# krlong014/PySolvers

Hardware: AMD Instinct MI355X
Metric: CG iterations/sec + SpMV GB/s vs HBM roofline, 5-pt Laplacian N=10M (higher is better)
Workload: dtype f64

## Files before the change

### include/psk_lab.h

```cpp
#ifndef PSK_LAB_H
#define PSK_LAB_H

#include "psk.h"

#ifdef __cplusplus
extern "C" {
#endif

int psk_lab_occupy_begin(int32_t wgs, int32_t lds_bytes, double seconds);
int psk_lab_occupy_end(int32_t *timed_out);
int psk_lab_dispatch_probe(int32_t nwg, int32_t lds_bytes, double usec, int64_t *rec_out);
int psk_lab_occupy_xcc(int32_t *counts);
int psk_lab_trisolve_workers(const psk_prec *M, int32_t which, int32_t *enrolled, int32_t *grid);
int psk_lab_trisolve_plan(int64_t n, const int32_t *rowptr, const int32_t *colidx, const double *vals, int32_t upper,
                          int32_t unit, const int32_t *nat, int32_t num_cus, int64_t syncfree_waves, int32_t *schedule,
                          double *est, int64_t *info);
int psk_lab_dist_plan(int64_t n_global, const int64_t *row_starts, int32_t P, int32_t rank, const int64_t *rowptr,
                      const int32_t *colidx, int32_t *lcol, int64_t *halo, int64_t *nhalo, int32_t *pack, int64_t *npack,
                      int64_t *peers, int32_t *npeers);
int psk_lab_amg_gs_pair(psk_prec *M, int32_t set, int32_t *levels_on, int32_t *levels_eligible);
int psk_lab_spmv_rotate(const psk_csr *A, const double *const *xs, double *const *ys, int32_t nbuf, int32_t reps,
                        int32_t dot, double *avg_ms);
int psk_lab_spmv_after_write(const psk_csr *A, double *x, double *y, const double *src, double *scratch,
                             int32_t target, int32_t reps, int32_t dot, double *avg_ms);
int psk_lab_cheby_ab(const psk_prec *M, const double *v, int32_t reps, double *fused_ms, double *pieces_ms);
int psk_lab_pcg_stagger(int32_t *blocks, int32_t *ring);
int psk_lab_pcg_staggers(const psk_csr *A, const psk_prec *M, int32_t *on);
int psk_lab_pcg_flush_schedule(int32_t S, int64_t nv, int64_t tile, int64_t k, int32_t in_spmv, int32_t *blk,
                               int64_t *first_last);
int psk_lab_pcg_flush(int64_t n, int64_t k, int32_t stag, double *x, const double *ring, const double *alphas);
#define PSK_LAB_SOLVER_PCG 0
#define PSK_LAB_SOLVER_GMRES 1
#define PSK_LAB_SOLVER_VCYCLE 2
#define PSK_LAB_SOLVER_BICGSTAB 3
#define PSK_LAB_LAYOUT_GEN 1
#define PSK_LAB_LAYOUT_OWN_X 2
#define PSK_LAB_LAYOUT_DEV_IO 4
int psk_lab_solver_layout(int32_t solver, int64_t n, int64_t ncols, int64_t maxiter, int64_t restart, int32_t flags,
                          int32_t P, int64_t *offsets, int32_t *count, int64_t *bytes);
int psk_lab_gmres_internals(const psk_csr *A, int64_t maxiter, int32_t restart, int32_t gen, int32_t cols, double *Q,
                            double *H, double *R, double *CS, double *g, double *y, double *state);
int psk_lab_gmres_prefill(psk_csr *A, int64_t maxiter, int32_t restart, int32_t gen, int32_t byte);
int psk_lab_ilu0_timing(double *out);
#ifdef __cplusplus
}
#endif

#endif
```

### pysolvers_amd/_native.py

```python
import atexit
import ctypes
import os
import sys

import numpy as np

_HERE = os.path.dirname(os.path.abspath(__file__))
LIB_PATH = os.environ.get("PSK_LIBRARY", os.path.join(_HERE, "_lib", "libpsk.so"))

PSK_OK = 0
PSK_ERR_ARG, PSK_ERR_HIP, PSK_ERR_RCCL, PSK_ERR_ALLOC, PSK_ERR_UNSUPPORTED = -1, -2, -3, -4, -5
ABI_VERSION = 4
PSK_CONVERGED, PSK_MAXITER, PSK_BREAKDOWN, PSK_TRUE_RESID_FAIL = 0, 1, 2, 3
PSK_EXIT_NONE, PSK_EXIT_TOLERANCE, PSK_EXIT_ARNOLDI_BREAKDOWN, PSK_EXIT_MAXITER, PSK_EXIT_DOT_BREAKDOWN = 0, 1, 2, 3, 4
PSK_HOST, PSK_DEVICE = 0, 1
PSK_VCYCLE_X0_GIVEN = 1
PSK_PREC_IDENTITY, PSK_PREC_JACOBI, PSK_PREC_ILU, PSK_PREC_AMG, PSK_PREC_DENSE, PSK_PREC_CHEBYSHEV = 0, 1, 2, 3, 4, 5
PSK_LAYOUT_CSR, PSK_LAYOUT_SLICED, PSK_LAYOUT_SLICED_WIDE, PSK_LAYOUT_SLICED_DICT, PSK_LAYOUT_DIAG = 0, 1, 2, 3, 4
PSK_UNIQUE_ID_BYTES = 128
PSK_SPGEMM_ROW_CAP = 1024

STATUS_NAMES = {PSK_CONVERGED: "converged", PSK_MAXITER: "maxiter", PSK_BREAKDOWN: "breakdown",
                PSK_TRUE_RESID_FAIL: "true residual above tolerance"}

# ... 55 lines not shown
                                                   ctypes.POINTER(I32), ctypes.POINTER(F64), ctypes.POINTER(F64)]),
    "psk_prec_trisolve_grid_info": (ctypes.c_int, [P, I32, ctypes.POINTER(I64)]),
    "psk_trisolve_grid_plan": (ctypes.c_int, [I64, P, P, P, I32, ctypes.POINTER(I64)]),
    "psk_prec_info": (ctypes.c_int, [P, ctypes.POINTER(I32)] + [ctypes.POINTER(I64)] * 5),
    "psk_mm_info": (ctypes.c_int, [ctypes.c_char_p] + [ctypes.POINTER(I64)] * 3),
    "psk_mm_read": (ctypes.c_int, [ctypes.c_char_p, P, P, P, ctypes.POINTER(I64)]),
    "psk_csr_create_mm": (ctypes.c_int, [ctypes.c_char_p, PP]),
    "psk_sa_aggregate": (ctypes.c_int, [I64, P, P, P, F64, P, ctypes.POINTER(I64), P]),
    "psk_csr_matmat": (ctypes.c_int, [P, P, PP]),
    "psk_csr_transpose": (ctypes.c_int, [P, PP]),
    "psk_sa_prolongator": (ctypes.c_int, [P, P, I64, P, F64, I32, PP]),
    "psk_csr_ilu0": (ctypes.c_int, [P, PP]),
    "psk_prec_create_ilu0": (ctypes.c_int, [P, PP]),
    "psk_pcg": (ctypes.c_int, [P, P, P, P, ctypes.POINTER(PskCtl), ctypes.POINTER(PskResult), P, I32]),
    "psk_gmres": (ctypes.c_int, [P, P, P, P, ctypes.POINTER(PskCtl), ctypes.POINTER(PskResult), P, I32]),
    "psk_bicgstab": (ctypes.c_int, [P, P, P, P, ctypes.POINTER(PskCtl), ctypes.POINTER(PskResult), P, I32]),
    "psk_vcycle": (ctypes.c_int, [P, P, P, ctypes.POINTER(PskCtl), ctypes.POINTER(PskResult), P, I32, I32]),
    "psk_comm_unique_id": (ctypes.c_int, [P]),
    "psk_comm_init": (ctypes.c_int, [I32, I32, P, PP]),
    "psk_comm_destroy": (ctypes.c_int, [P]),
    "psk_comm_init_dry": (ctypes.c_int, [I32, I32, PP]),
    "psk_comm_init_host": (ctypes.c_int, [I32, I32, ctypes.c_char_p, PP]),
    "psk_comm_mailbox": (ctypes.c_int, [P, ctypes.c_char_p]),
    "psk_comm_mailbox_check": (ctypes.c_int, [P, I32]),
    "psk_csr_create_fd2d_dist": (ctypes.c_int, [F64, F64, I64, P, PP, ctypes.POINTER(I64),
                                                ctypes.POINTER(I64)]),
    "psk_csr_create_dist": (ctypes.c_int, [I64, P, P, P, P, P, PP]),
    "psk_csr_halo_cols": (ctypes.c_int, [P, P, ctypes.POINTER(I64)]),
    "psk_csr_halo_peers": (ctypes.c_int, [P, P, P, P, P, ctypes.POINTER(I32)]),
    "psk_csr_halo_pack": (ctypes.c_int, [P, P, P]),
    "psk_fd2d_dist_plan": (ctypes.c_int, [I64, I32, I32] + [ctypes.POINTER(I64)] * 5),
}


LAB_PATH = os.path.join(os.path.dirname(LIB_PATH), "libpsk_lab.so")
LAB_SIGNATURES = {
    "psk_lab_occupy_begin": (ctypes.c_int, [I32, I32, F64]),
    "psk_lab_occupy_end": (ctypes.c_int, [ctypes.POINTER(I32)]),
    "psk_lab_occupy_xcc": (ctypes.c_int, [ctypes.POINTER(I32)]),
    "psk_lab_dispatch_probe": (ctypes.c_int, [I32, I32, F64, P]),
    "psk_lab_trisolve_workers": (ctypes.c_int, [P, I32, ctypes.POINTER(I32), ctypes.POINTER(I32)]),
    "psk_lab_trisolve_plan": (ctypes.c_int, [I64, P, P, P, I32, I32, P, I32, I64, ctypes.POINTER(I32),
                                             ctypes.POINTER(F64), ctypes.POINTER(I64)]),
    "psk_lab_dist_plan": (ctypes.c_int, [I64, P, I32, I32, P, P, P, P, ctypes.POINTER(I64), P, ctypes.POINTER(I64), P,
                                         ctypes.POINTER(I32)]),
    "psk_lab_amg_gs_pair": (ctypes.c_int, [P, I32, ctypes.POINTER(I32), ctypes.POINTER(I32)]),
    "psk_lab_spmv_rotate": (ctypes.c_int, [P, ctypes.POINTER(P), ctypes.POINTER(P), I32, I32, I32, ctypes.POINTER(F64)]),
    "psk_lab_cheby_ab": (ctypes.c_int, [P, P, I32, ctypes.POINTER(F64), ctypes.POINTER(F64)]),
    "psk_lab_spmv_after_write": (ctypes.c_int, [P, P, P, P, P, I32, I32, I32, ctypes.POINTER(F64)]),
    "psk_lab_pcg_stagger": (ctypes.c_int, [ctypes.POINTER(I32), ctypes.POINTER(I32)]),
    "psk_lab_pcg_staggers": (ctypes.c_int, [P, P, ctypes.POINTER(I32)]),
    "psk_lab_pcg_flush_schedule": (ctypes.c_int, [I32, I64, I64, I64, I32, ctypes.POINTER(I32), ctypes.POINTER(I64)]),
    "psk_lab_pcg_flush": (ctypes.c_int, [I64, I64, I32, P, P, P]),
    "psk_lab_solver_layout": (ctypes.c_int, [I32, I64, I64, I64, I64, I32, I32, ctypes.POINTER(I64),
                                            ctypes.POINTER(I32), ctypes.POINTER(I64)]),
    "psk_lab_gmres_internals": (ctypes.c_int, [P, I64, I32, I32, I32, P, P, P, P, P, P, P]),
    "psk_lab_gmres_prefill": (ctypes.c_int, [P, I64, I32, I32, I32]),
    "psk_lab_ilu0_timing": (ctypes.c_int, [ctypes.POINTER(F64)]),
}
_lab = None


def load_lab():
    global _lab
    if _lab is None:
        if not os.path.exists(LAB_PATH):
            raise ImportError("libpsk_lab.so not found at %s (make -C pysolvers_amd/csrc)" % LAB_PATH)
        lab = ctypes.CDLL(LAB_PATH)
        for name, (res, args) in LAB_SIGNATURES.items():
            fn = getattr(lab, name)
            fn.restype = res
            fn.argtypes = args
        _lab = lab
    return _lab


def prec_info(h):
    k = I32()
    v = [I64() for _ in range(5)]
    check(lib.psk_prec_info(h, ctypes.byref(k), *[ctypes.byref(x) for x in v]), "psk_prec_info")
    return dict(kind=k.value, n=v[0].value, nnz_l=v[1].value, nnz_u=v[2].value, levels_l=v[3].value,
                levels_u=v[4].value)


def handle_array(hs):
    arr = (ctypes.c_void_p * max(len(hs), 1))()
    for i, h in enumerate(hs):
        arr[i] = h.value if isinstance(h, ctypes.c_void_p) else h
    return ctypes.cast(arr, PP), arr


def fd2d_dist_plan(m, nranks, rank):
    v = [I64() for _ in range(5)]
    check(lib.psk_fd2d_dist_plan(m, nranks, rank, *[ctypes.byref(x) for x in v]), "psk_fd2d_dist_plan")
    return tuple(x.value for x in v)


class PskError(RuntimeError):

    def __init__(self, code, where, text):
        super().__init__("%s failed (%d): %s" % (where, code, text))
        self.code = code


def _pin_runtime():
    import importlib.util
# ... 59 lines not shown
```

### pysolvers_amd/csrc/lab.hip

```cpp
#include "amg.hpp"
#include "dist.hpp"
#include "trisolve.hpp"
#include "pcg_state.hpp"
#include "solve_loop.hpp"
#include "../../include/psk_lab.h"

#include <algorithm>
#include <chrono>
#include <string>

namespace psk {

__global__ __launch_bounds__(1024) void occupy_kernel(uint32_t *flag, int64_t *started, uint64_t ticks,
                                                      int32_t *timed_out) {
    extern __shared__ unsigned char occ_lds[];
    if (threadIdx.x == 0) {
        occ_lds[0] = 1;
        __hip_atomic_fetch_add(started, (int64_t)1, __ATOMIC_RELAXED, __HIP_MEMORY_SCOPE_SYSTEM);
        const uint32_t xcc = __builtin_amdgcn_s_getreg((3 << 11) | 20) & 7u;
        __hip_atomic_fetch_add(reinterpret_cast<uint32_t *>(timed_out) + 32 + xcc, 1u, __ATOMIC_RELAXED,
                               __HIP_MEMORY_SCOPE_AGENT);
    }
    const uint64_t t0 = __builtin_amdgcn_s_memrealtime();
    while (__hip_atomic_load(flag, __ATOMIC_RELAXED, __HIP_MEMORY_SCOPE_AGENT) == 0) {
        if (__builtin_amdgcn_s_memrealtime() - t0 > ticks) {
            if (threadIdx.x == 0) atomicOr(timed_out, 1);
            break;
        }
        __builtin_amdgcn_s_sleep(8);
    }
}
__global__ void occupy_release_kernel(uint32_t *flag) {
    __hip_atomic_store(flag, 1u, __ATOMIC_RELAXED, __HIP_MEMORY_SCOPE_AGENT);
}

namespace {
struct Occupier {
    hipStream_t s = nullptr;
    uint32_t *dw = nullptr;
    int64_t *started = nullptr;
    bool active = false;
};
Occupier g_occ;
}

}

extern "C" int psk_lab_occupy_begin(int32_t wgs, int32_t lds_bytes, double seconds) {
    using namespace psk;
    Context *c;
    PSK_TRY(ctx(&c));
    if (g_occ.active) return fail(PSK_ERR_ARG, "psk_lab_occupy_begin: already active");
    if (wgs < 1 || lds_bytes < 16 || lds_bytes > 160 * 1024 || seconds <= 0)
        return fail(PSK_ERR_ARG, "psk_lab_occupy_begin: bad arguments");
    if (!g_occ.s) {
        PSK_HIP(hipStreamCreateWithFlags(&g_occ.s, hipStreamNonBlocking));
        PSK_HIP(hipMalloc(&g_occ.dw, 128 * sizeof(uint32_t)));
// ... 220 lines not shown
    const int64_t n = A->n;
    const unsigned g = (unsigned)((n + 511) / 512);
    double *dst = target == 1 ? x : scratch;
    rc = launch_spmv(A, mode, x, y, nullptr, nullptr, pp, nullptr, c->stream);
    for (int32_t r = 0; r < reps && rc == PSK_OK; ++r) {
        if (target > 0) {
            hipLaunchKernelGGL(lab_copy_kernel, dim3(g), dim3(256), 0, c->stream, n, src, dst);
            if (hipGetLastError() != hipSuccess) rc = fail(PSK_ERR_HIP, "lab copy");
        }
        if (rc == PSK_OK)
            rc = launch_spmv(A, mode, x, y, nullptr, nullptr, pp, nullptr, c->stream, ea[(size_t)r], eb[(size_t)r]);
    }
    double tot = 0.0;
    if (rc == PSK_OK && hipStreamSynchronize(c->stream) != hipSuccess) rc = fail(PSK_ERR_HIP, "sync");
    for (int32_t r = 0; r < reps && rc == PSK_OK; ++r) {
        float ms = 0.f;
        if (hipEventElapsedTime(&ms, ea[(size_t)r], eb[(size_t)r]) != hipSuccess) rc = fail(PSK_ERR_HIP, "event time");
        tot += ms;
    }
    (void)hipStreamSynchronize(c->stream);
    for (int32_t r = 0; r < reps; ++r) {
        (void)hipEventDestroy(ea[(size_t)r]);
        (void)hipEventDestroy(eb[(size_t)r]);
    }
    part.release();
    if (rc == PSK_OK) *avg_ms = tot / reps;
    return rc;
}

extern "C" int psk_lab_pcg_stagger(int32_t *blocks, int32_t *ring) {
    if (blocks) *blocks = psk::kPcgStagger;
    if (ring) *ring = psk::kPcgDefer;
    return PSK_OK;
}

extern "C" int psk_lab_pcg_staggers(const psk_csr *A, const psk_prec *M, int32_t *on) {
    if (!A || !on) return psk::fail(PSK_ERR_ARG, "psk_lab_pcg_staggers: NULL argument");
    *on = psk::pcg_staggers(A, M) ? 1 : 0;
    return PSK_OK;
}

extern "C" int psk_lab_pcg_flush_schedule(int32_t S, int64_t nv, int64_t tile, int64_t k, int32_t in_spmv,
                                          int32_t *blk, int64_t *first_last) {
    using namespace psk;
    if (S < 1 || nv < 1 || tile < 0 || tile >= nv || k < 0 || !blk || !first_last)
        return fail(PSK_ERR_ARG, "psk_lab_pcg_flush_schedule: bad arguments");
    *blk = pcg_block_of_tile(tile, nv, S);
    const PcgPend pd = pcg_flush_pending(S, *blk, k, in_spmv != 0);
    first_last[0] = pd.first;
    first_last[1] = pd.last;
    return PSK_OK;
}

extern "C" int psk_lab_pcg_flush(int64_t n, int64_t k, int32_t stag, double *x, const double *ring,
                                 const double *alphas) {
    using namespace psk;
    if (n < 1 || k < 1 || !x || !ring || !alphas) return fail(PSK_ERR_ARG, "psk_lab_pcg_flush: bad arguments");
    if (stag && kPcgStagger == 0) return fail(PSK_ERR_UNSUPPORTED, "psk_lab_pcg_flush: built without the staggered flush");
    Context *c;
    PSK_TRY(ctx(&c));
    const size_t vec = ((size_t)n * 8 + 255) / 256 * 256, al = ((size_t)k * 8 + 255) / 256 * 256;
    DevBuf buf;
    PSK_TRY(buf.ensure((kPcgDefer + 1) * vec + al));
    char *d = buf.as<char>();
    double *dx = reinterpret_cast<double *>(d), *da = reinterpret_cast<double *>(d + (kPcgDefer + 1) * vec);
    PRing pr;
    for (int t = 0; t < kPcgDefer; ++t) pr.b[t] = reinterpret_cast<double *>(d + (size_t)(t + 1) * vec);
    int rc = PSK_OK;
    if (hipMemcpyAsync(dx, x, (size_t)n * 8, hipMemcpyHostToDevice, c->stream) != hipSuccess ||
        hipMemcpyAsync(da, alphas, (size_t)k * 8, hipMemcpyHostToDevice, c->stream) != hipSuccess)
        rc = fail(PSK_ERR_HIP, "psk_lab_pcg_flush: copy");
    for (int t = 0; t < kPcgDefer && rc == PSK_OK; ++t)
        if (hipMemcpyAsync(pr.b[t], ring + (size_t)t * (size_t)n, (size_t)n * 8, hipMemcpyHostToDevice, c->stream) != hipSuccess)
            rc = fail(PSK_ERR_HIP, "psk_lab_pcg_flush: copy");
    if (rc == PSK_OK) rc = launch_pcg_flush(n, dx, pr, da, k, stag != 0, c->stream);
    if (rc == PSK_OK && hipMemcpyAsync(x, dx, (size_t)n * 8, hipMemcpyDeviceToHost, c->stream) != hipSuccess)
        rc = fail(PSK_ERR_HIP, "psk_lab_pcg_flush: copy back");
    if (hipStreamSynchronize(c->stream) != hipSuccess && rc == PSK_OK) rc = fail(PSK_ERR_HIP, "psk_lab_pcg_flush: sync");
    buf.release();
    return rc;
}

extern "C" int psk_lab_solver_layout(int32_t solver, int64_t n, int64_t ncols, int64_t maxiter, int64_t restart,
                                     int32_t flags, int32_t P, int64_t *offsets, int32_t *count, int64_t *bytes) {
    using namespace psk;
    if (n < 0 || ncols < 0 || maxiter < 0 || restart < 0 || P < 1 || !offsets || !count || !bytes)
        return fail(PSK_ERR_ARG, "psk_lab_solver_layout: bad arguments");
    std::vector<int64_t> log;
    const bool gen = (flags & PSK_LAB_LAYOUT_GEN) != 0;
    if (solver == PSK_LAB_SOLVER_PCG) pcg_layout_probe(n, ncols, maxiter, gen, (flags & PSK_LAB_LAYOUT_OWN_X) != 0, P, &log, bytes);
    else if (solver == PSK_LAB_SOLVER_GMRES) gmres_layout_probe(n, maxiter, restart, gen, &log, bytes);
    else if (solver == PSK_LAB_SOLVER_BICGSTAB) bicgstab_layout_probe(n, maxiter, gen, &log, bytes);
    else if (solver == PSK_LAB_SOLVER_VCYCLE) vcycle_layout_probe(n, maxiter, (flags & PSK_LAB_LAYOUT_DEV_IO) != 0, &log, bytes);
    else return fail(PSK_ERR_ARG, "psk_lab_solver_layout: unknown solver");
    if ((size_t)*count < log.size()) return fail(PSK_ERR_ARG, "psk_lab_solver_layout: offsets too short");
    *count = (int32_t)log.size();
    for (size_t i = 0; i < log.size(); ++i) offsets[i] = log[i];
    return PSK_OK;
}

extern "C" int psk_lab_gmres_internals(const psk_csr *A, int64_t maxiter, int32_t restart, int32_t gen, int32_t cols,
                                       double *Q, double *H, double *R, double *CS, double *g, double *y,
                                       double *state) {
    using namespace psk;
    if (!A || cols < 0) return fail(PSK_ERR_ARG, "psk_lab_gmres_internals: bad arguments");
    GmresView v;
// ... 41 lines not shown
```

### pysolvers_amd/csrc/spmv.hpp

```cpp
#pragma once
#include "psk_internal.hpp"

#include <hip/hip_ext.h>

#include <type_traits>

namespace psk {

constexpr int kSlice = kBlock;

__device__ __forceinline__ bool same_bits(double a, double b) {
    return __double_as_longlong(a) == __double_as_longlong(b);
}

struct SpmvLaunch {
    const double *x;
    double *y;
    const double *aux_d, *aux_q;
    GridSum gs;
    const int32_t *done;
    hipStream_t s;
    hipEvent_t ev0, ev1;
    bool rev;
    int64_t nwg;
};
struct SpmvFlush;
int launch_spmv_csr(const psk_csr *A, int mode, const SpmvLaunch &L);
int launch_spmv_sliced(const psk_csr *A, int mode, const SpmvLaunch &L);
int launch_spmv_diag(const psk_csr *A, int mode, const SpmvLaunch &L, const SpmvFlush *flush);

int sliced_build(psk_csr *A, hipStream_t s, bool force, bool pack, bool use_dict, bool force_dict);
void sliced_free(psk_csr *A);
int sliced_shape(const psk_csr *A, hipStream_t s, int32_t *width, int32_t *span);
int diag_build(psk_csr *A, hipStream_t s, bool force);
void diag_free(psk_csr *A);

template <int V>
using SpmvInt = std::integral_constant<int, V>;
template <class F>
int spmv_for_mode(int mode, F &&f) {
    switch (mode) {
    case kSpmvPlain: f(SpmvInt<kSpmvPlain>{}); break;
    case kSpmvDot: f(SpmvInt<kSpmvDot>{}); break;
    case kSpmvJacobiDot: f(SpmvInt<kSpmvJacobiDot>{}); break;
    case kSpmvPlainDot: f(SpmvInt<kSpmvPlainDot>{}); break;
    case kSpmvResid: f(SpmvInt<kSpmvResid>{}); break;
    case kSpmvAdd: f(SpmvInt<kSpmvAdd>{}); break;
    default:
        return fail(PSK_ERR_ARG, "unknown spmv mode");
    }
    PSK_HIP(hipGetLastError());
    return PSK_OK;
}


__device__ __forceinline__ int32_t ld_stream(const int32_t *p) { return __builtin_nontemporal_load(p); }
__device__ __forceinline__ double ld_stream(const double *p) { return __builtin_nontemporal_load(p); }

template <int MODE>
__device__ __forceinline__ bool spmv_publishes(const GridSum &gs) {
    return MODE != kSpmvPlain && MODE != kSpmvAdd && (MODE != kSpmvResid || gs.out != nullptr);
}
template <int MODE>
__device__ __forceinline__ uint32_t spmv_begin(const GridSum &gs, GridSumTile<1> &L, int64_t t) {
    return spmv_publishes<MODE>(gs) ? gridsum_tile_begin<1>(gs, L, t) : 0u;
}
__device__ __forceinline__ void spmv_publish(const GridSum &gs, GridSumTile<1> &L, double acc, uint32_t ticket,
                                             int64_t t) {
    const double ws = wave_total(acc);
    gridsum_tile_publish<1>(gs, L, &ws, ticket, t);
}

template <int MODE>
__device__ __forceinline__ double spmv_row_value(bool has, double sum, double eq, double &acc) {
    const double yv = MODE == kSpmvResid ? eq - sum : MODE == kSpmvAdd ? eq + sum : sum;
    acc = 0.0;
    if (has && MODE != kSpmvPlain && MODE != kSpmvAdd) acc = MODE == kSpmvResid ? yv * yv : eq * sum;
    return yv;
}
template <int MODE>
__device__ __forceinline__ void spmv_store_row(bool has, int64_t row, double yv, double *__restrict__ y) {
    if (!has) return;
// ... 57 lines not shown
```

### pysolvers_amd/csrc/spmv_diag.hip

```cpp
#include "spmv.hpp"
#include "pcg_state.hpp"

#include <algorithm>
#include <climits>

namespace psk {

static __device__ int32_t g_spmv_never_done = 0;

constexpr int kDiagMax = 8;
constexpr int kDiagTpw = 2;
struct DiagDesc {
    int32_t d[kDiagMax];
    double v[kDiagMax];
    int64_t lo, hi;
    int64_t ncols;
    int32_t K, jd;
};

__device__ __forceinline__ int64_t diag_col(const DiagDesc &dd, int64_t n, int64_t row, int j) {
    int64_t c = row + dd.d[j];
    c += c < 0 ? dd.lo : (c >= n ? dd.hi : 0);
    return c < 0 ? 0 : (c >= dd.ncols ? dd.ncols - 1 : c);
}
// ... 107 lines not shown
            const double t = sum + dd.v[j] * xv[q][j];
            sum = ((mk[q] >> j) & 1u) ? t : sum;
        }
        if (MODE == kSpmvDot) {
            double d = 0.0;
            bool found = false;
#pragma unroll
            for (int j = 0; j < KM; ++j) {
                const bool here = j == dd.jd && ((mk[q] >> j) & 1u);
                d = here ? xv[q][j] : d;
                found = found || here;
            }
            if (!found && has) d = x[row];
            eq[q] = d;
        }
        yv[q] = spmv_row_value<MODE>(has, sum, eq[q], acc[q]);
    }
    if (pub) spmv_publish_multi<TPW>(gs, gsl, acc, ticket, tl, tv);
#pragma unroll
    for (int q = 0; q < TPW; ++q) {
        const int64_t row = tl[q] * kSlice + tid;
        spmv_store_row<MODE>(tv[q] && row < n, row, yv[q], y);
    }
}


typedef double dv2u __attribute__((ext_vector_type(2), aligned(8)));
__device__ __forceinline__ dv2 ldu2(const double *p) {
    const dv2u v = *reinterpret_cast<const dv2u *>(p);
    return dv2{v.x, v.y};
}
__device__ __forceinline__ dv2 ldu2nt(const double *p) {
    const dv2u v = __builtin_nontemporal_load(reinterpret_cast<const dv2u *>(p));
    return dv2{v.x, v.y};
}
__device__ __forceinline__ void stu2(double *p, dv2 v) { *reinterpret_cast<dv2u *>(p) = dv2u{v.x, v.y}; }
__device__ __forceinline__ void stu2nt(double *p, dv2 v) {
    __builtin_nontemporal_store(dv2u{v.x, v.y}, reinterpret_cast<dv2u *>(p));
}

__device__ __forceinline__ double lane_f64(double x, int l) {
    return __hiloint2double(__builtin_amdgcn_readlane(__double2hiint(x), l),
                            __builtin_amdgcn_readlane(__double2loint(x), l));
}
__device__ __forceinline__ void diag_pair_totals(double v, double &t0, double &t1) {
    v += dpp_f64<0xB1>(v);
    v += dpp_f64<0x141>(v);
    v += dpp_f64<0x104>(v);
    t0 = ((lane_f64(v, 0) + lane_f64(v, 8)) + lane_f64(v, 16)) + lane_f64(v, 24);
    t1 = ((lane_f64(v, 32) + lane_f64(v, 40)) + lane_f64(v, 48)) + lane_f64(v, 56);
}

struct PairFix {
    int64_t c0, c1;
    bool bad;
};
__device__ __forceinline__ dv2 diag_pair_x(const DiagDesc &dd, int64_t n, int64_t r, int64_t d,
                                           const double *__restrict__ x, PairFix &f) {
    int64_t c0 = r + d, c1 = c0 + 1;
    c0 += c0 < 0 ? dd.lo : (c0 >= n ? dd.hi : 0);
    c1 += c1 < 0 ? dd.lo : (c1 >= n ? dd.hi : 0);
    f.bad = !(c1 == c0 + 1 && c0 >= 0 && c1 < dd.ncols);
    f.c0 = c0 < 0 ? 0 : (c0 >= dd.ncols ? dd.ncols - 1 : c0);
    f.c1 = c1 < 0 ? 0 : (c1 >= dd.ncols ? dd.ncols - 1 : c1);
    const int64_t a = c0 < 0 ? 0 : (c0 > dd.ncols - 2 ? dd.ncols - 2 : c0);
    return ldu2(x + a);
}
__device__ __forceinline__ void diag_pair_fix(dv2 &v, const PairFix &f, const double *__restrict__ x) {
    if (f.bad) {
        v.x = x[f.c0];
        v.y = x[f.c1];
    }
}

__host__ __device__ inline uint32_t spmv_flush_octets_before(const SpmvFlush &f, uint32_t o) {
    if (f.mul == 0) return o > f.ost ? o - f.ost : 0;
    return (uint32_t)(((uint64_t)o * f.mul) >> 16);
}
__device__ __forceinline__ const SpmvFlush &spmv_flush_arg(const SpmvFlush &f) { return f; }

template <int S>
__device__ __forceinline__ void spmv_flush_tile(const SpmvFlush &fl, uint32_t f, int64_t n) {
    const int64_t k = fl.k;
    const int blk = (int)(k % S);
    const PcgPend pd = pcg_flush_pending(S, blk, k, true);
    const int q = (int)(k - pd.first);
    const bool x0 = pd.first == 0;
    const int64_t i = ((int64_t)blk * pcg_block_tiles(fl.nv, S) + f) * kVecTile + 2 * threadIdx.x;
    double *__restrict__ x = fl.x;
    if (i + 1 < n) {
        dv2 xo{0.0, 0.0};
        if (!x0) xo = ld2nt(x + i);
        dv2 pp[S];
#pragma unroll
        for (int t = 1; t <= S; ++t)
            if (t <= q) pp[t - 1] = ld2nt(fl.pr.b[(k - t) % kPcgDefer] + i);
#pragma unroll
        for (int t = S; t >= 1; --t)
            if (t <= q) {
                const double a = fl.alphas[k - t];
                xo.x = xo.x + a * pp[t - 1].x;
                xo.y = xo.y + a * pp[t - 1].y;
            }
        st2nt(x + i, xo);
    } else if (i < n) {
        x[i] = pcg_catch_up(x0 ? 0.0 : x[i], &fl.pr, pd.first, k, fl.alphas, i);
    }
}

template <int MODE, int NB, typename... FLUSH>
__global__ __launch_bounds__(kBlock, (MODE != kSpmvPlain && MODE != kSpmvDot) ? 4 : 8) void spmv_diagp_kernel(
    int64_t n, const uint8_t *__restrict__ mask, DiagDesc dd, const double *__restrict__ x, double *__restrict__ y,
    const double *__restrict__ aux_d, const double *__restrict__ aux_q, GridSum gs, const int32_t *__restrict__ done,
    TileMap tm, int64_t ntiles, FLUSH... flush) {
    constexpr int KM = 5;
    constexpr int H = 2;
    constexpr bool FL = sizeof...(FLUSH) == 1;
    static_assert(sizeof...(FLUSH) <= 1 && (!FL || (MODE == kSpmvDot && kPcgStagger > 0)),
                  "the flush role rides on the PCG loop's launch only");
    static_assert(NB == 1 || NB == 2, "the 5-diagonal DPP orders");
    constexpr int JD = NB == 1 ? 0 : 2, JM1 = NB == 1 ? 3 : 1, JP1 = NB == 1 ? 4 : 3;
    constexpr int GD = NB == 1 ? 0 : 1;
    constexpr int TPB = kWaves;
    constexpr bool JX = MODE == kSpmvJacobiDot;
    constexpr bool EQ = MODE == kSpmvResid || MODE == kSpmvAdd || MODE == kSpmvJacobiDot || MODE == kSpmvPlainDot;
    const int32_t dnv = (done ? done : &g_spmv_never_done)[spmv_vzero()];
    const int lane = threadIdx.x & 63;
    const int wave = __builtin_amdgcn_readfirstlane(threadIdx.x >> 6);
    int64_t sidx = blockIdx.x, scnt = gridDim.x;
    if constexpr (FL) {
        const SpmvFlush &fl = spmv_flush_arg(flush...);
        const uint32_t o = blockIdx.x >> 3, fb = spmv_flush_octets_before(fl, o);
        if (spmv_flush_octets_before(fl, o + 1) != fb) {
            const uint32_t f = fb * 8 + (blockIdx.x & 7);
            if (f >= fl.nfl || __builtin_amdgcn_readfirstlane(dnv) != 0) return;
            spmv_flush_tile<kPcgStagger>(fl, f, n);
            return;
        }
        sidx = (int64_t)(o - fb) * 8 + (blockIdx.x & 7);
        scnt = (gs.nt + TPB - 1) / TPB;
        if (sidx >= scnt) return;
    }
    const int64_t grp = tile_of_index(tm, sidx, scnt);
    const int64_t t = grp * TPB + wave;
    const bool tv = t < ntiles;
    const int64_t tl = tv ? t : ntiles - 1;
    const int64_t r0 = tl * kSlice;
    uint32_t mk[H];
    dv2 xv[H][3], dg[H][3], eq[H];
    PairFix fx[H][3];
    double xe, de = 1.0;
#pragma unroll
    for (int h = 0; h < H; ++h) {
        const int64_t row = r0 + 128 * h + 2 * lane;
        mk[h] = __builtin_nontemporal_load(reinterpret_cast<const uint16_t *>(mask + row));
    }
#pragma unroll
    for (int h = 0; h < H; ++h) {
        const int64_t row = r0 + 128 * h + 2 * lane;
        int g = 0;
#pragma unroll
        for (int j = 0; j < KM; ++j) {
            if (j == JM1 || j == JP1) continue;
            xv[h][g] = diag_pair_x(dd, n, row, dd.d[j], x, fx[h][g]);
            if (JX) dg[h][g] = diag_pair_x(dd, n, row, dd.d[j], aux_d, fx[h][g]);
            ++g;
        }
        eq[h] = dv2{0.0, 0.0};
        if (EQ) eq[h] = ldu2(aux_q + (row + 1 < n ? row : (n >= 2 ? n - 2 : 0)));
    }
    {
        const int64_t er = lane == 0 ? r0 - 1 : (lane == 63 ? r0 + 128 * H : r0 + 2 * lane);
        const int64_t c = diag_col_off(dd, n, er, 0);
        xe = x[c];
        if (JX) de = aux_d[c];
    }
    constexpr bool PUB = MODE != kSpmvPlain && MODE != kSpmvAdd;
    const bool pub = PUB && spmv_publishes<MODE>(gs);
    uint32_t ticket = 0;
    if (pub && tv && gs.grp_log2 >= 0 && lane == 0)
        ticket = gridsum_draw(gridsum_counter(gs, gridsum_group_of(tl, gs.grp_log2)));
    if (__builtin_amdgcn_readfirstlane(dnv) != 0) {
#pragma unroll
        for (int h = 0; h < H; ++h) {
            __asm__ volatile("" ::"v"(mk[h]));
#pragma unroll
            for (int g = 0; g < 3; ++g) {
                __asm__ volatile("" ::"v"(xv[h][g].x), "v"(xv[h][g].y));
                if (JX) __asm__ volatile("" ::"v"(dg[h][g].x), "v"(dg[h][g].y));
            }
            if (EQ) __asm__ volatile("" ::"v"(eq[h].x), "v"(eq[h].y));
        }
        __asm__ volatile("" ::"v"(xe), "v"(de));
        if (pub && tv && gs.grp_log2 >= 0 && lane == 0)
            __hip_atomic_fetch_sub(gridsum_counter(gs, gridsum_group_of(tl, gs.grp_log2)), 1u, __ATOMIC_RELAXED,
                                   __HIP_MEMORY_SCOPE_AGENT);
        return;
    }
    if constexpr (FL) {
        const SpmvFlush &fl = spmv_flush_arg(flush...);
        const uint32_t ot = gridDim.x >> 3;
        if (pub && threadIdx.x == 0 && sidx == 0 &&
            ((gridDim.x & 7) != 0 || (scnt + 7) / 8 != (int64_t)(ot - spmv_flush_octets_before(fl, ot))))
            atomicOr(gs.err, 2);
    } else {
        if (pub && threadIdx.x == 0 && blockIdx.x == 0 && (gs.nt + TPB - 1) / TPB != gridDim.x) atomicOr(gs.err, 2);
    }
#pragma unroll
    for (int h = 0; h < H; ++h)
#pragma unroll
        for (int g = 0; g < 3; ++g) {
            diag_pair_fix(xv[h][g], fx[h][g], x);
            if (JX) {
                diag_pair_fix(dg[h][g], fx[h][g], aux_d);
                xv[h][g].x = dg[h][g].x * xv[h][g].x;
                xv[h][g].y = dg[h][g].y * xv[h][g].y;
            }
        }
    if (JX) xe = de * xe;
    double xl[H], xr[H];
    const double a63 = lane_f64(xv[0][GD].y, 63), b0 = lane_f64(xv[1][GD].x, 0);
    xl[0] = wave_shift1<true>(xv[0][GD].y, xe);
    xr[0] = wave_shift1<false>(xv[0][GD].x, b0);
    xl[1] = wave_shift1<true>(xv[1][GD].y, a63);
    xr[1] = wave_shift1<false>(xv[1][GD].x, xe);
    double acc[H];
    dv2 yv[H];
#pragma unroll
    for (int h = 0; h < H; ++h) {
        const int64_t row = r0 + 128 * h + 2 * lane;
        double c0[KM], c1[KM];
        int g = 0;
#pragma unroll
        for (int j = 0; j < KM; ++j) {
            if (j == JM1) {
                c0[j] = xl[h];
                c1[j] = xv[h][GD].x;
            } else if (j == JP1) {
                c0[j] = xv[h][GD].y;
                c1[j] = xr[h];
            } else {
                c0[j] = xv[h][g].x;
                c1[j] = xv[h][g].y;
                ++g;
            }
        }
        const uint32_t m0 = mk[h] & 0xffu, m1 = mk[h] >> 8;
        double s0 = 0.0, s1 = 0.0;
#pragma unroll
        for (int j = 0; j < KM; ++j) {
            const double u0 = s0 + dd.v[j] * c0[j], u1 = s1 + dd.v[j] * c1[j];
            s0 = ((m0 >> j) & 1u) ? u0 : s0;
            s1 = ((m1 >> j) & 1u) ? u1 : s1;
        }
        const bool has0 = tv && row < n, has1 = tv && row + 1 < n;
        double e0 = eq[h].x, e1 = eq[h].y;
        if (EQ && row + 1 >= n) {
            e0 = eq[h].y;
            e1 = 0.0;
        }
        if (MODE == kSpmvDot) {
            const bool f0 = (m0 >> JD) & 1u, f1 = (m1 >> JD) & 1u;
            e0 = f0 ? c0[JD] : 0.0;
            e1 = f1 ? c1[JD] : 0.0;
            if (!f0 && has0) e0 = x[row];
            if (!f1 && has1) e1 = x[row + 1];
        }
// ... 214 lines not shown
            if (dd.d[i] == d) return no("repeated column in a row");
        dd.d[j] = (int32_t)d;
        dd.v[j] = vals[(size_t)j];
        if (d == 0) dd.jd = j;
        dmin = std::min(dmin, d);
    }
    const int64_t halo = A->ncols - n;
    dd.lo = halo > 0 ? n - dmin : 0;
    dd.hi = halo > 0 && halo == -2 * dmin ? -dmin : 0;
    dd.ncols = A->ncols;
    uint8_t *mask = nullptr;
    if (hipMalloc(&mask, (size_t)nt * kSlice) != hipSuccess) {
        (void)hipGetLastError();
        return force ? fail(PSK_ERR_ALLOC, "diagonal layout: hipMalloc") : PSK_OK;
    }
    PSK_HIP(hipMemsetAsync(dbad, 0, sizeof(int32_t), s));
    hipLaunchKernelGGL(diag_detect_kernel, dim3((unsigned)nt), dim3(kBlock), 0, s, n, A->rowptr, A->colidx, A->vals, dd,
                       mask, nt * kSlice, dbad);
    int32_t bad = 0;
    hipError_t e = hipGetLastError();
    if (e == hipSuccess) e = hipMemcpyAsync(&bad, dbad, sizeof(int32_t), hipMemcpyDeviceToHost, s);
    if (e == hipSuccess) e = hipStreamSynchronize(s);
    if (e != hipSuccess || bad) {
        (void)hipFree(mask);
        if (e != hipSuccess) return fail(PSK_ERR_HIP, std::string("diagonal layout: ") + hipGetErrorString(e));
        return no("an entry off the diagonals or with another value");
    }
    sliced_free(A);
    diag_free(A);
    A->dg_mask = mask;
    A->dg_K = K;
    A->dg_jd = dd.jd;
    for (int j = 0; j < kDiagMax; ++j) {
        A->dg_d[j] = j < K ? dd.d[j] : 0;
        A->dg_v[j] = j < K ? dd.v[j] : 0.0;
    }
    A->dg_lo = dd.lo;
    A->dg_hi = dd.hi;
    return PSK_OK;
}

static int diag_nb(const psk_csr *A) {
    if (!A->dg_mask || A->dg_K != 5) return 0;
    if (A->dg_d[0] == 0 && A->dg_d[3] == -1 && A->dg_d[4] == 1) return 1;
    if (A->dg_d[2] == 0 && A->dg_d[1] == -1 && A->dg_d[3] == 1) return 2;
    return 0;
}

static bool diag_pair_rows(const psk_csr *A) { return diag_nb(A) != 0 && A->n >= 2 && A->ncols >= 2; }

bool pcg_init_diag_eligible(const psk_csr *A) { return !A->comm && A->n > 0 && diag_nb(A) != 0; }
bool spmv_flush_eligible(const psk_csr *A) { return !A->comm && diag_pair_rows(A); }

static uint32_t spmv_flush_grid(SpmvFlush &fl, int64_t nwgp) {
    constexpr int S = kPcgStagger > 0 ? kPcgStagger : 1;
    const int64_t per = pcg_block_tiles(fl.nv, S), t0 = (fl.k % S) * per;
    const int64_t nf = std::min(fl.nv, t0 + per) - t0;
    fl.nfl = nf > 0 ? (uint32_t)nf : 0;
    if (fl.nfl == 0) return 0;
    const int64_t ost = (nwgp + 7) / 8, ofl = (nf + 7) / 8;
    if ((ost + ofl + 2) * 8 > (int64_t)INT32_MAX) return 0;
    fl.ost = (uint32_t)ost;
    fl.ofl = (uint32_t)ofl;
    uint32_t ot = (uint32_t)(ost + ofl);
    const int64_t mul = (ofl * 65536 + ot - 1) / ot;
    fl.mul = (uint32_t)std::min<int64_t>(std::max<int64_t>(mul, 1), 65535);
    while (ot < (uint32_t)(ost + ofl + 2) * 2 &&
           (spmv_flush_octets_before(fl, ot) < fl.ofl || ot - spmv_flush_octets_before(fl, ot) < fl.ost))
        ++ot;
    if (spmv_flush_octets_before(fl, ot) < fl.ofl || ot - spmv_flush_octets_before(fl, ot) != fl.ost) {
        fl.mul = 0;
        ot = (uint32_t)(ost + ofl);
    }
    return ot * 8;
}

int launch_spmv_diag(const psk_csr *A, int mode, const SpmvLaunch &L, const SpmvFlush *flush) {
    const DiagDesc dd = diag_desc(A);
    const dim3 bd(kBlock);
    const int nb = diag_nb(A);
    if (diag_pair_rows(A)) {
        const int64_t nwgp = (L.nwg + kWaves - 1) / kWaves;
        const dim3 gdp((unsigned)nwgp);
        const TileMap tmp = tile_map_for(nwgp, true, L.rev);
#if PSK_PCG_STAGGER_ON
        if (flush) {
            SpmvFlush fl = *flush;
            const uint32_t grid = spmv_flush_grid(fl, nwgp);
            if (fl.nfl > 0) {
                if (grid == 0) return fail(PSK_ERR_UNSUPPORTED, "launch_spmv: grid too large for the flush role");
                if (nb == 1)
                    hipExtLaunchKernelGGL((spmv_diagp_kernel<kSpmvDot, 1, SpmvFlush>), dim3(grid), bd, 0, L.s, L.ev0,
                                          L.ev1, 0, A->n, A->dg_mask, dd, L.x, L.y, L.aux_d, L.aux_q, L.gs, L.done, tmp,
                                          L.nwg, fl);
                else
                    hipExtLaunchKernelGGL((spmv_diagp_kernel<kSpmvDot, 2, SpmvFlush>), dim3(grid), bd, 0, L.s, L.ev0,
                                          L.ev1, 0, A->n, A->dg_mask, dd, L.x, L.y, L.aux_d, L.aux_q, L.gs, L.done, tmp,
                                          L.nwg, fl);
                PSK_HIP(hipGetLastError());
                return PSK_OK;
            }
        }
#endif
        return spmv_for_mode(mode, [&](auto m) {
            constexpr int M = decltype(m)::value;
            if (nb == 1)
                hipExtLaunchKernelGGL((spmv_diagp_kernel<M, 1>), gdp, bd, 0, L.s, L.ev0, L.ev1, 0, A->n, A->dg_mask, dd,
                                      L.x, L.y, L.aux_d, L.aux_q, L.gs, L.done, tmp, L.nwg);
            else
                hipExtLaunchKernelGGL((spmv_diagp_kernel<M, 2>), gdp, bd, 0, L.s, L.ev0, L.ev1, 0, A->n, A->dg_mask, dd,
                                      L.x, L.y, L.aux_d, L.aux_q, L.gs, L.done, tmp, L.nwg);
        });
    }
    const int64_t nwgd = (L.nwg + kDiagTpw - 1) / kDiagTpw;
    const dim3 gdd((unsigned)(nwgd > 0 ? nwgd : 1));
    const TileMap tmd = tile_map_for(nwgd, true, L.rev);
    return spmv_for_mode(mode, [&](auto m) {
        constexpr int M = decltype(m)::value;
        auto one_row = [&](auto kmc, auto nbc) {
            hipExtLaunchKernelGGL((spmv_diag_kernel<M, decltype(kmc)::value, kDiagTpw, decltype(nbc)::value>), gdd, bd,
                                  0, L.s, L.ev0, L.ev1, 0, A->n, A->dg_mask, dd, L.x, L.y, L.aux_d, L.aux_q, L.gs,
                                  L.done, tmd, L.nwg);
        };
        if (nb == 1) one_row(SpmvInt<5>{}, SpmvInt<1>{});
        else if (nb == 2) one_row(SpmvInt<5>{}, SpmvInt<2>{});
        else if (A->dg_K <= 3) one_row(SpmvInt<3>{}, SpmvInt<0>{});
        else if (A->dg_K <= 5) one_row(SpmvInt<5>{}, SpmvInt<0>{});
        else one_row(SpmvInt<8>{}, SpmvInt<0>{});
    });
}

int launch_pcg_init_diag(const psk_csr *A, const double *b, double xs, double *p, double *Ap, double *out3,
                         const PcgInitFin &fin, hipStream_t s) {
    if (!pcg_init_diag_eligible(A)) return fail(PSK_ERR_ARG, "launch_pcg_init_diag: not eligible");
    Context *c;
    PSK_TRY(ctx(&c));
    const int64_t nwg = (A->n + kSlice - 1) / kSlice, nwgd = (nwg + kDiagTpw - 1) / kDiagTpw;
    GridSum gs;
    PSK_TRY(gridsum_prepare(c, nwg, 3, out3, &gs));
    const DiagDesc dd = diag_desc(A);
    const TileMap tmd = tile_map_for(nwgd, true);
    if (diag_nb(A) == 1)
        hipLaunchKernelGGL(pcg_init_diag_kernel<1>, dim3((unsigned)nwgd), dim3(kBlock), 0, s, A->n, A->dg_mask, dd, b, xs,
                           p, Ap, gs, fin, tmd, nwg);
    else
        hipLaunchKernelGGL(pcg_init_diag_kernel<2>, dim3((unsigned)nwgd), dim3(kBlock), 0, s, A->n, A->dg_mask, dd, b, xs,
                           p, Ap, gs, fin, tmd, nwg);
    PSK_HIP(hipGetLastError());
    return PSK_OK;
}

}
```

Measured before the change: 7562.

## Add opt-in stacked tile mapping sharing x stencil loads via LDS in diag SpMV

Adds an optional tile remapping in which the four waves of a workgroup handle vertically stacked slices of a 2D stencil. The off-diagonal x reads (±m offsets) can then be served from a shared LDS slab instead of HBM. Separately, the per-lane boundary-fix state is replaced with a wave ballot mask held in scalar registers, and fix-up column indices are recomputed on demand to cut vector register use. The stacking path is compiled out by default via a macro, and a lab entry point exposes the tile rule for testing.

```diff
diff --git a/include/psk_lab.h b/include/psk_lab.h
--- a/include/psk_lab.h
+++ b/include/psk_lab.h
@@ -29,6 +29,7 @@
 int psk_lab_pcg_flush_schedule(int32_t S, int64_t nv, int64_t tile, int64_t k, int32_t in_spmv, int32_t *blk,
                                int64_t *first_last);
 int psk_lab_pcg_flush(int64_t n, int64_t k, int32_t stag, double *x, const double *ring, const double *alphas);
+int psk_lab_spmv_stack(int64_t nt, int64_t m, int32_t sharded, int32_t *ng, int32_t *s, int64_t *tiles);
 #define PSK_LAB_SOLVER_PCG 0
 #define PSK_LAB_SOLVER_GMRES 1
 #define PSK_LAB_SOLVER_VCYCLE 2
diff --git a/pysolvers_amd/_native.py b/pysolvers_amd/_native.py
--- a/pysolvers_amd/_native.py
+++ b/pysolvers_amd/_native.py
@@ -131,6 +131,7 @@
     "psk_lab_pcg_staggers": (ctypes.c_int, [P, P, ctypes.POINTER(I32)]),
     "psk_lab_pcg_flush_schedule": (ctypes.c_int, [I32, I64, I64, I64, I32, ctypes.POINTER(I32), ctypes.POINTER(I64)]),
     "psk_lab_pcg_flush": (ctypes.c_int, [I64, I64, I32, P, P, P]),
+    "psk_lab_spmv_stack": (ctypes.c_int, [I64, I64, I32, ctypes.POINTER(I32), ctypes.POINTER(I32), P]),
     "psk_lab_solver_layout": (ctypes.c_int, [I32, I64, I64, I64, I64, I32, I32, ctypes.POINTER(I64),
                                             ctypes.POINTER(I32), ctypes.POINTER(I64)]),
     "psk_lab_gmres_internals": (ctypes.c_int, [P, I64, I32, I32, I32, P, P, P, P, P, P, P]),
diff --git a/pysolvers_amd/csrc/lab.hip b/pysolvers_amd/csrc/lab.hip
--- a/pysolvers_amd/csrc/lab.hip
+++ b/pysolvers_amd/csrc/lab.hip
@@ -3,6 +3,7 @@
 #include "trisolve.hpp"
 #include "pcg_state.hpp"
 #include "solve_loop.hpp"
+#include "spmv.hpp"
 #include "../../include/psk_lab.h"
 
 #include <algorithm>
@@ -329,6 +330,21 @@
     return PSK_OK;
 }
 
+extern "C" int psk_lab_spmv_stack(int64_t nt, int64_t m, int32_t sharded, int32_t *ng, int32_t *s, int64_t *tiles) {
+    using namespace psk;
+    if (nt < 1 || !ng || !s) return fail(PSK_ERR_ARG, "psk_lab_spmv_stack: bad arguments");
+    const SpmvStack st = spmv_stack_rule(nt, m, sharded != 0);
+    *ng = st.ng;
+    *s = st.s;
+    if (tiles) {
+        const int64_t nwg = (nt + kWaves - 1) / kWaves;
+        if (nwg > (int64_t)INT32_MAX) return fail(PSK_ERR_ARG, "psk_lab_spmv_stack: too many tiles");
+        for (int64_t g = 0; g < nwg; ++g)
+            for (int w = 0; w < kWaves; ++w) tiles[g * kWaves + w] = spmv_stack_tile(st, (uint32_t)g, w);
+    }
+    return PSK_OK;
+}
+
 extern "C" int psk_lab_pcg_flush(int64_t n, int64_t k, int32_t stag, double *x, const double *ring,
                                  const double *alphas) {
     using namespace psk;
diff --git a/pysolvers_amd/csrc/spmv.hpp b/pysolvers_amd/csrc/spmv.hpp
--- a/pysolvers_amd/csrc/spmv.hpp
+++ b/pysolvers_amd/csrc/spmv.hpp
@@ -28,6 +28,20 @@
 int launch_spmv_csr(const psk_csr *A, int mode, const SpmvLaunch &L);
 int launch_spmv_sliced(const psk_csr *A, int mode, const SpmvLaunch &L);
 int launch_spmv_diag(const psk_csr *A, int mode, const SpmvLaunch &L, const SpmvFlush *flush);
+
+#ifndef PSK_SPMV_STACK
+#define PSK_SPMV_STACK 0
+#endif
+struct SpmvStack {
+    int32_t ng;
+    int32_t s;
+};
+__host__ __device__ inline int64_t spmv_stack_tile(const SpmvStack &st, uint32_t g, int w) {
+    if (g >= (uint32_t)st.ng) return (int64_t)g * 4 + w;
+    const uint32_t B = g / (uint32_t)st.s, i = g - B * (uint32_t)st.s;
+    return ((int64_t)B * 4 + w) * st.s + i;
+}
+SpmvStack spmv_stack_rule(int64_t nt, int64_t m, bool sharded);
 
 int sliced_build(psk_csr *A, hipStream_t s, bool force, bool pack, bool use_dict, bool force_dict);
 void sliced_free(psk_csr *A);
diff --git a/pysolvers_amd/csrc/spmv_diag.hip b/pysolvers_amd/csrc/spmv_diag.hip
--- a/pysolvers_amd/csrc/spmv_diag.hip
+++ b/pysolvers_amd/csrc/spmv_diag.hip
@@ -183,24 +183,28 @@
 }
 
 struct PairFix {
-    int64_t c0, c1;
-    bool bad;
+    uint64_t bad;
 };
-__device__ __forceinline__ dv2 diag_pair_x(const DiagDesc &dd, int64_t n, int64_t r, int64_t d,
-                                           const double *__restrict__ x, PairFix &f) {
+__device__ __forceinline__ const double *diag_pair_at(const DiagDesc &dd, int64_t n, int64_t r, int64_t d,
+                                                      const double *__restrict__ x, PairFix &f) {
     int64_t c0 = r + d, c1 = c0 + 1;
     c0 += c0 < 0 ? dd.lo : (c0 >= n ? dd.hi : 0);
     c1 += c1 < 0 ? dd.lo : (c1 >= n ? dd.hi : 0);
-    f.bad = !(c1 == c0 + 1 && c0 >= 0 && c1 < dd.ncols);
-    f.c0 = c0 < 0 ? 0 : (c0 >= dd.ncols ? dd.ncols - 1 : c0);
-    f.c1 = c1 < 0 ? 0 : (c1 >= dd.ncols ? dd.ncols - 1 : c1);
+    f.bad = __builtin_amdgcn_ballot_w64(!(c1 == c0 + 1 && c0 >= 0 && c1 < dd.ncols));
+    __asm__ volatile("" : "+s"(f.bad));
     const int64_t a = c0 < 0 ? 0 : (c0 > dd.ncols - 2 ? dd.ncols - 2 : c0);
-    return ldu2(x + a);
-}
-__device__ __forceinline__ void diag_pair_fix(dv2 &v, const PairFix &f, const double *__restrict__ x) {
-    if (f.bad) {
-        v.x = x[f.c0];
-        v.y = x[f.c1];
+    return x + a;
+}
+__device__ __forceinline__ dv2 diag_pair_x(const DiagDesc &dd, int64_t n, int64_t r, int64_t d,
+                                           const double *__restrict__ x, PairFix &f) {
+    return ldu2(diag_pair_at(dd, n, r, d, x, f));
+}
+__device__ __forceinline__ void diag_pair_fix(dv2 &v, const PairFix &f, const DiagDesc &dd, int64_t n, int64_t r,
+                                              int64_t d, const double *__restrict__ x) {
+    if ((f.bad >> (threadIdx.x & 63)) & 1u) {
+        __asm__ volatile("" : "+v"(r));
+        v.x = x[diag_col_off(dd, n, r, d)];
+        v.y = x[diag_col_off(dd, n, r + 1, d)];
     }
 }
 
@@ -239,12 +243,19 @@
     }
 }
 
+__device__ __forceinline__ bool stack_in_lds(bool stk, int wave, bool lower, int i, int dl, int ulim) {
+    const int li = lower ? i - dl : i + dl;
+    return stk && (lower ? wave > 0 : wave < kWaves - 1) && li >= 0 && li + 1 < kSlice && (lower || i < ulim);
+}
+
 template <int MODE, int NB, typename... FLUSH>
 __global__ __launch_bounds__(kBlock, (MODE != kSpmvPlain && MODE != kSpmvDot) ? 4 : 8) void spmv_diagp_kernel(
     int64_t n, const uint8_t *__restrict__ mask, DiagDesc dd, const double *__restrict__ x, double *__restrict__ y,
     const double *__restrict__ aux_d, const double *__restrict__ aux_q, GridSum gs, const int32_t *__restrict__ done,
-    TileMap tm, int64_t ntiles, FLUSH... flush) {
+    TileMap tm, int64_t ntiles, SpmvStack st, FLUSH... flush) {
     constexpr int KM = 5;
+    constexpr bool ST = PSK_SPMV_STACK && MODE == kSpmvDot;
+    constexpr int GL = NB == 1 ? 1 : 0;
     constexpr int H = 2;
     constexpr bool FL = sizeof...(FLUSH) == 1;
     static_assert(sizeof...(FLUSH) <= 1 && (!FL || (MODE == kSpmvDot && kPcgStagger > 0)),
@@ -273,10 +284,22 @@
         if (sidx >= scnt) return;
     }
     const int64_t grp = tile_of_index(tm, sidx, scnt);
-    const int64_t t = grp * TPB + wave;
+    int64_t t = grp * TPB + wave;
+    bool stk = false;
+    int dl = 0;
+    if constexpr (ST) {
+        stk = grp < st.ng;
+        t = spmv_stack_tile(st, (uint32_t)grp, wave);
+        dl = dd.d[NB == 1 ? 2 : 4] - kSlice * st.s;
+    }
     const bool tv = t < ntiles;
     const int64_t tl = tv ? t : ntiles - 1;
     const int64_t r0 = tl * kSlice;
+    int ulim = 0;
+    if constexpr (ST) {
+        const int64_t u = n - 1 - dd.d[NB == 1 ? 2 : 4] - r0;
+        ulim = u < 0 ? 0 : (u > kSlice ? kSlice : (int)u);
+    }
     uint32_t mk[H];
     dv2 xv[H][3], dg[H][3], eq[H];
     PairFix fx[H][3];
@@ -287,19 +310,27 @@
         mk[h] = __builtin_nontemporal_load(reinterpret_cast<const uint16_t *>(mask + row));
     }
 #pragma unroll
-    for (int h = 0; h < H; ++h) {
-        const int64_t row = r0 + 128 * h + 2 * lane;
-        int g = 0;
-#pragma unroll
-        for (int j = 0; j < KM; ++j) {
-            if (j == JM1 || j == JP1) continue;
-            xv[h][g] = diag_pair_x(dd, n, row, dd.d[j], x, fx[h][g]);
-            if (JX) dg[h][g] = diag_pair_x(dd, n, row, dd.d[j], aux_d, fx[h][g]);
-            ++g;
-        }
-        eq[h] = dv2{0.0, 0.0};
-        if (EQ) eq[h] = ldu2(aux_q + (row + 1 < n ? row : (n >= 2 ? n - 2 : 0)));
-    }
+    for (int ph = 0; ph < (ST ? 2 : 1); ++ph)
+#pragma unroll
+        for (int h = 0; h < H; ++h) {
+            const int64_t row = r0 + 128 * h + 2 * lane;
+            int g = 0;
+#pragma unroll
+            for (int j = 0; j < KM; ++j) {
+                if (j == JM1 || j == JP1) continue;
+                if (!ST || (ph == 0) == (g == GD)) {
+                    const double *a = diag_pair_at(dd, n, row, dd.d[j], x, fx[h][g]);
+                    if (!(ST && g != GD && stack_in_lds(stk, wave, g == GL, 128 * h + 2 * lane, dl, ulim)))
+                        xv[h][g] = ldu2(a);
+                    if (JX) dg[h][g] = diag_pair_x(dd, n, row, dd.d[j], aux_d, fx[h][g]);
+                }
+                ++g;
+            }
+            if (ph == 0) {
+                eq[h] = dv2{0.0, 0.0};
+                if (EQ) eq[h] = ldu2(aux_q + (row + 1 < n ? row : (n >= 2 ? n - 2 : 0)));
+            }
+        }
     {
         const int64_t er = lane == 0 ? r0 - 1 : (lane == 63 ? r0 + 128 * H : r0 + 2 * lane);
         const int64_t c = diag_col_off(dd, n, er, 0);
@@ -337,13 +368,38 @@
     } else {
         if (pub && threadIdx.x == 0 && blockIdx.x == 0 && (gs.nt + TPB - 1) / TPB != gridDim.x) atomicOr(gs.err, 2);
     }
+    if constexpr (ST) {
+        __shared__ __attribute__((aligned(16))) double slab[TPB][kSlice];
+        if (stk) {
+#pragma unroll
+            for (int h = 0; h < H; ++h)
+                *reinterpret_cast<dv2 *>(&slab[wave][128 * h + 2 * lane]) = xv[h][GD];
+            __builtin_amdgcn_fence(__ATOMIC_RELEASE, "workgroup", "local");
+            __builtin_amdgcn_s_barrier();
+            __builtin_amdgcn_fence(__ATOMIC_ACQUIRE, "workgroup", "local");
+#pragma unroll
+            for (int h = 0; h < H; ++h)
+#pragma unroll
+                for (int g = 0; g < 3; ++g) {
+                    if (g == GD) continue;
+                    const int i = 128 * h + 2 * lane;
+                    if (stack_in_lds(true, wave, g == GL, i, dl, ulim)) {
+                        const double *sl = &slab[g == GL ? wave - 1 : wave + 1][g == GL ? i - dl : i + dl];
+                        xv[h][g].x = sl[0];
+                        xv[h][g].y = sl[1];
+                    }
+                }
+        }
+    }
 #pragma unroll
     for (int h = 0; h < H; ++h)
 #pragma unroll
         for (int g = 0; g < 3; ++g) {
-            diag_pair_fix(xv[h][g], fx[h][g], x);
+            constexpr int JG[3] = {NB == 1 ? 0 : 0, NB == 1 ? 1 : 2, 4 - 2 * (NB == 1)};
+            const int64_t row = r0 + 128 * h + 2 * lane;
+            diag_pair_fix(xv[h][g], fx[h][g], dd, n, row, dd.d[JG[g]], x);
             if (JX) {
-                diag_pair_fix(dg[h][g], fx[h][g], aux_d);
+                diag_pair_fix(dg[h][g], fx[h][g], dd, n, row, dd.d[JG[g]], aux_d);
                 xv[h][g].x = dg[h][g].x * xv[h][g].x;
                 xv[h][g].y = dg[h][g].y * xv[h][g].y;
             }
@@ -664,6 +720,21 @@
 bool pcg_init_diag_eligible(const psk_csr *A) { return !A->comm && A->n > 0 && diag_nb(A) != 0; }
 bool spmv_flush_eligible(const psk_csr *A) { return !A->comm && diag_pair_rows(A); }
 
+SpmvStack spmv_stack_rule(int64_t nt, int64_t m, bool sharded) {
+    if (!PSK_SPMV_STACK || sharded || m < 1 || nt < 1) return SpmvStack{0, 0};
+    const int64_t s = (m + kSlice / 2) / kSlice;
+    if (s < 1 || nt / (4 * s) < 1 || nt > (int64_t)INT32_MAX) return SpmvStack{0, 0};
+    return SpmvStack{(int32_t)(nt / (4 * s) * s), (int32_t)s};
+}
+
+static SpmvStack diag_stack(const psk_csr *A, int mode, int64_t nt) {
+    const int nb = diag_nb(A);
+    if (mode != kSpmvDot || nb == 0) return SpmvStack{0, 0};
+    const int64_t lo = A->dg_d[nb == 1 ? 1 : 0], up = A->dg_d[nb == 1 ? 2 : 4];
+    if (lo != -up) return SpmvStack{0, 0};
+    return spmv_stack_rule(nt, up, A->comm != nullptr || A->ncols != A->n);
+}
+
 static uint32_t spmv_flush_grid(SpmvFlush &fl, int64_t nwgp) {
     constexpr int S = kPcgStagger > 0 ? kPcgStagger : 1;
     const int64_t per = pcg_block_tiles(fl.nv, S), t0 = (fl.k % S) * per;
@@ -695,6 +766,7 @@
         const int64_t nwgp = (L.nwg + kWaves - 1) / kWaves;
         const dim3 gdp((unsigned)nwgp);
         const TileMap tmp = tile_map_for(nwgp, true, L.rev);
+        const SpmvStack st = diag_stack(A, mode, L.nwg);
 #if PSK_PCG_STAGGER_ON
         if (flush) {
             SpmvFlush fl = *flush;
@@ -704,11 +776,11 @@
                 if (nb == 1)
                     hipExtLaunchKernelGGL((spmv_diagp_kernel<kSpmvDot, 1, SpmvFlush>), dim3(grid), bd, 0, L.s, L.ev0,
                                           L.ev1, 0, A->n, A->dg_mask, dd, L.x, L.y, L.aux_d, L.aux_q, L.gs, L.done, tmp,
-                                          L.nwg, fl);
+                                          L.nwg, st, fl);
                 else
                     hipExtLaunchKernelGGL((spmv_diagp_kernel<kSpmvDot, 2, SpmvFlush>), dim3(grid), bd, 0, L.s, L.ev0,
                                           L.ev1, 0, A->n, A->dg_mask, dd, L.x, L.y, L.aux_d, L.aux_q, L.gs, L.done, tmp,
-                                          L.nwg, fl);
+                                          L.nwg, st, fl);
                 PSK_HIP(hipGetLastError());
                 return PSK_OK;
             }
@@ -718,10 +790,10 @@
             constexpr int M = decltype(m)::value;
             if (nb == 1)
                 hipExtLaunchKernelGGL((spmv_diagp_kernel<M, 1>), gdp, bd, 0, L.s, L.ev0, L.ev1, 0, A->n, A->dg_mask, dd,
-                                      L.x, L.y, L.aux_d, L.aux_q, L.gs, L.done, tmp, L.nwg);
+                                      L.x, L.y, L.aux_d, L.aux_q, L.gs, L.done, tmp, L.nwg, st);
             else
                 hipExtLaunchKernelGGL((spmv_diagp_kernel<M, 2>), gdp, bd, 0, L.s, L.ev0, L.ev1, 0, A->n, A->dg_mask, dd,
-                                      L.x, L.y, L.aux_d, L.aux_q, L.gs, L.done, tmp, L.nwg);
+                                      L.x, L.y, L.aux_d, L.aux_q, L.gs, L.done, tmp, L.nwg, st);
         });
     }
     const int64_t nwgd = (L.nwg + kDiagTpw - 1) / kDiagTpw;
```

New measurement: 7539. Within noise of the previous version (-0.3%).
